# lukedan/libfluid

Hardware: AMD Instinct MI355X
Metric: particle_steps_per_sec (higher is better)
Workload: dtype f32

## Files before the change

libfluid_amd/csrc/common.h:

```cpp
#pragma once

#include <hip/hip_runtime.h>
#include <stdint.h>

#include <string>
#include <vector>

#include "../../include/libfluid_amd.h"

hipError_t lfa_pool_malloc(void **p, size_t bytes);
hipError_t lfa_pool_free(void *p);
void lfa_pool_nosync_begin();
void lfa_pool_nosync_end();
template <typename T> inline hipError_t lfa_hip_malloc(T **p, size_t bytes) { return lfa_pool_malloc((void **)p, bytes); }
#define hipMalloc(p, n) lfa_hip_malloc((p), (n))
#define hipFree(p) lfa_pool_free((void *)(p))
struct lfa_stream_set;
lfa_stream_set *lfa_pool_take_set(int device);
void lfa_pool_park_set(lfa_stream_set *q);

#define LFA_TILE 8
#define LFA_TILE_CELLS 512
#define LFA_HALO 10
#define LFA_HALO_CELLS 1000
// ... 34 lines not shown
	int mg_no_closed = 0;
	int mg_no_tagged = 0;
};

struct lfa_sim {
	int device = 0;
	lfa_knobs knobs;
	hipStream_t stream = nullptr;
	hipStream_t stream2 = nullptr;
	hipEvent_t ev_fork = nullptr, ev_join = nullptr;
	hipStream_t stream3 = nullptr;
	hipEvent_t ev_cfork = nullptr, ev_cjoin = nullptr;
	bool overlap_correction = true;
	bool corr_in_flight = false;
	bool counts_fresh = false;
	bool move_pending = false;
	bool corr_begun = false;
	bool corr_undo_valid = false;
	uint32_t *corr_ovf = nullptr;
	int corr_parts_tiles = 0;
	GridDims g{};
	size_t nc = 0, ncp = 0;
	lfa_params prm{};
	std::string err;

	size_t np = 0, pcap = 0;
	ParticleSoA pb[2];
	int cur = 0;
	uint32_t *rank = nullptr;
	bool binned = false;
// ... 352 lines not shown

int lfa_exclusive_scan_u32(lfa_sim *s, const uint32_t *in, uint32_t *out, size_t n, uint32_t *total_dev);
enum {
	LFA_PIN_SOURCE_TOTAL = 96,
	LFA_PIN_SEED_ACCEPTED = 97,
	LFA_PIN_SEED_OWNED = 98,
	LFA_PIN_RESIDENT = 99,
	LFA_PIN_SOURCE_TOTAL_ALL = 104,
	LFA_PIN_SOURCE_KEPT = 105,
	LFA_PIN_SAMPLE_OWNED = 106,
	LFA_PIN_SAMPLE_OUTSIDE = 107,
};
int lfa_scan_total(lfa_sim *s, const uint32_t *in, uint32_t *out, size_t n, uint32_t *total_dev, int slot, size_t *total);

int lfa_particles_alloc(lfa_sim *s, size_t n);
int lfa_hash_particles_impl(lfa_sim *s, bool counts_done);
int lfa_particles_materialize(lfa_sim *s);
int lfa_c_home_restore(lfa_sim *s);
int lfa_c_home_ensure(lfa_sim *s, size_t n);
int lfa_ensure_io(lfa_sim *s, size_t bytes);
int lfa_slab_download_slots(lfa_sim *s, const uint32_t **slot);
int lfa_sample_velocity_launch(lfa_sim *s, hipStream_t stream, const double *xyz, size_t n, const uint32_t *tile_rule, int z_lo, int z_hi,
                               double *velocity, uint8_t *types, uint32_t *counts_dev);
int lfa_sample_refresh(lfa_sim *s, const char *who, size_t room_bytes, const uint32_t **tile_rule, void **room, int *z_lo, int *z_hi);
int lfa_pcg_alloc(lfa_sim *s);
int lfa_number_unknowns(lfa_sim *s);

__host__ __device__ inline int lfa_stage_index(int hx, int hy, int hz) {
	return (unsigned)(hx - 1) < 8u ? (hx - 1) + 8 * (hy + 10 * hz) : 800 + (hx ? 100 : 0) + hy + 10 * hz;
}
__host__ __device__ inline int lfa_stage_source(int o) {
// ... 64 lines not shown
```

libfluid_amd/csrc/core.hip:

```cpp
#include <math.h>

#include <algorithm>
#include <stdarg.h>
#include <stdio.h>
#include <string.h>

#include <mutex>

#include "common.h"
#include "pcg.h"
#include "stream_set.h"

static thread_local std::string g_create_error;

int lfa_fail(lfa_sim *s, int code, const char *fmt, ...) {
	char buf[512];
	va_list ap;
	va_start(ap, fmt);
	vsnprintf(buf, sizeof buf, fmt, ap);
	va_end(ap);
	if (s) s->err = buf;
	else g_create_error = buf;
	return code;
}
// ... 1033 lines not shown

int lfa_particles_materialize(lfa_sim *s) {
	if (!s->vc_pending) return LFA_OK;
	LFA_TRY(lfa_corr_commit(s));
	s->vc_pending = false;
	LFA_HIP(s, hipSetDevice(s->device));
	const size_t n = s->np_live;
	if (!n) return LFA_OK;
	hipLaunchKernelGGL(k_gather_vc, dim3((unsigned)((n + 255) / 256)), dim3(256), 0, s->stream, n, s->pb[s->cur ^ 1], s->pb[s->cur],
	                   (const uint32_t *)s->vc_src, s->vc_with_c ? 1 : 0);
	LFA_LAUNCH_CHECK(s);
	return LFA_OK;
}

extern "C" int lfa_hash_particles(lfa_sim *s) { return lfa_hash_particles_impl(s, false); }
int lfa_hash_particles_impl(lfa_sim *s, bool counts_done) {
	if (!s) return LFA_E_INVALID;
	LFA_HIP(s, hipSetDevice(s->device));
	LFA_TRY(lfa_corr_commit(s));
	LFA_TRY(lfa_particles_materialize(s));
	const GridDims &g = s->g;
	const int nt = g.nt, L = g.ntx * g.nty;
	const size_t n = s->binned ? s->np_live : s->np;
	ParticleSoA &src = s->pb[s->cur], &dst = s->pb[s->cur ^ 1];
	const int own_lo = s->slab_lo * L, own_hi = s->slab_hi * L;
	const int all_lo = lfa_has_lo(s) ? own_lo - L : own_lo, all_hi = lfa_has_hi(s) ? own_hi + L : own_hi;

	if (!counts_done) {
		LFA_HIP(s, hipMemsetAsync(s->tile_count, 0, (size_t)(nt + 1) * 4, s->stream));
		if (n) {
			hipLaunchKernelGGL(k_tile_count, dim3((unsigned)((n + 256 * TC_CHUNKS - 1) / (256 * TC_CHUNKS))), dim3(256), 0, s->stream, src.key, n,
			                   s->tile_count, s->rank);
			LFA_LAUNCH_CHECK(s);
		}
	}
	LFA_TRY(lfa_exclusive_scan_u32(s, s->tile_count, s->tile_start, (size_t)nt + 1, nullptr));
	LFA_HIP(s, hipMemcpyAsync(s->h_pinned + 8, s->tile_start + nt, 4, hipMemcpyDeviceToHost, s->stream));

	hipLaunchKernelGGL(k_tile_flags, dim3((nt + 255) / 256), dim3(256), 0, s->stream, s->tile_count, s->tile_flag, nt);
	LFA_LAUNCH_CHECK(s);
	LFA_TRY(lfa_dist_exchange_tile_layers_u32(s, s->tile_flag));
	hipLaunchKernelGGL(k_fill_i32, dim3((nt + 255) / 256), dim3(256), 0, s->stream, s->tile_pslot, nt, -1);
	LFA_LAUNCH_CHECK(s);
	const bool one_sync = !s->dist;
	if (one_sync) {
		uint32_t *tot = (uint32_t *)s->pcg_state + 8;
		LFA_TRY(compact_tiles_async(s, s->tile_flag, 0, nt, s->ptiles_all, s->tile_pslot, tot));
		LFA_HIP(s, hipMemsetAsync(s->tile_flag, 0, (size_t)(nt + 1) * 4, s->stream));
		hipLaunchKernelGGL(k_dilate_slots, dim3((nt + 255) / 256), dim3(256), 0, s->stream, (const int *)s->tile_pslot, s->tile_flag, g);
		LFA_LAUNCH_CHECK(s);
		LFA_TRY(compact_tiles_async(s, s->tile_flag, 0, nt, s->dtiles, nullptr, tot + 1));
		LFA_HIP(s, hipMemcpyAsync(s->h_pinned + 9, tot, 8, hipMemcpyDeviceToHost, s->stream));
		LFA_HIP(s, hipStreamSynchronize(s->stream));
		s->n_ptiles_all = (int)s->h_pinned[9];
		s->n_dtiles = (int)s->h_pinned[10];
		s->p_off = 0;
		s->n_ptiles = s->n_ptiles_all;
		s->n_own_first = s->n_own_last = s->n_ghost_lo = s->n_ghost_hi = 0;
		s->ptiles = s->ptiles_all;
	} else {
		uint32_t *tot = (uint32_t *)s->pcg_state + 20;
		LFA_TRY(compact_tiles_async(s, s->tile_flag, all_lo, all_hi, s->ptiles_all, s->tile_pslot, tot));
		int marks[4] = {own_lo, own_lo + L < own_hi ? own_lo + L : own_hi, own_hi - L > own_lo ? own_hi - L : own_lo, own_hi};
		int *didx = s->pcg_state + 12;
		LFA_HIP(s, hipMemcpyAsync(didx, marks, 16, hipMemcpyHostToDevice, s->stream));
		hipLaunchKernelGGL(k_gather_u32, dim3(1), dim3(64), 0, s->stream, s->tile_scan, didx, 4, tot + 1);
		LFA_LAUNCH_CHECK(s);
		LFA_HIP(s, hipMemsetAsync(s->tile_flag, 0, (size_t)(nt + 1) * 4, s->stream));
		hipLaunchKernelGGL(k_dilate_slots, dim3((nt + 255) / 256), dim3(256), 0, s->stream, (const int *)s->tile_pslot, s->tile_flag, g);
		LFA_LAUNCH_CHECK(s);
		if (own_lo > 0) LFA_HIP(s, hipMemsetAsync(s->tile_flag, 0, (size_t)own_lo * 4, s->stream));
		if (own_hi < nt) LFA_HIP(s, hipMemsetAsync(s->tile_flag + own_hi, 0, (size_t)(nt - own_hi) * 4, s->stream));
		LFA_TRY(lfa_dist_exchange_tile_layers_u32(s, s->tile_flag));
		LFA_TRY(compact_tiles_async(s, s->tile_flag, own_lo, own_hi, s->dtiles, nullptr, tot + 5));
		{
// ... 12 lines not shown
		s->p_off = vals[0];
		s->n_ptiles = vals[3] - vals[0];
		s->n_own_first = vals[1] - vals[0];
		s->n_own_last = vals[3] - vals[2];
		s->n_ghost_lo = s->p_off;
		s->n_ghost_hi = s->n_ptiles_all - vals[3];
		s->ptiles = s->ptiles_all + s->p_off;
		s->n_dtiles = (int)h[5];
		for (int w = 0; w < 4; ++w) s->n_halo[w] = (int)h[6 + w];
	}
	s->np_live = s->h_pinned[8];
	if (s->dist) s->np = s->np_live;
	s->holes = false;
	s->n_arrivals = 0;
	s->move_pending = false;
	if (n) {
		const dim3 sgrid((unsigned)((n + 255) / 256));
		const bool home = s->prm.simulation_method != LFA_APIC;
		if (home && !s->c_home_valid) {
			LFA_TRY(lfa_c_home_ensure(s, s->dist ? std::max<size_t>(s->pcap, (size_t)s->next_global_id) : s->pcap));
			hipLaunchKernelGGL(k_c_to_home, sgrid, dim3(256), 0, s->stream, n, src, s->c_home, s->c_home_cap);
			LFA_LAUNCH_CHECK(s);
			s->c_home_valid = true;
		} else if (!home && s->c_home_valid) {
			LFA_TRY(lfa_c_home_restore(s));
		}
		hipLaunchKernelGGL(k_tile_scatter, sgrid, dim3(256), 0, s->stream, n, src, dst, s->rank, s->tile_start, s->tile_count,
		                   s->binned ? 0 : 1, s->vc_src);
		LFA_LAUNCH_CHECK(s);
		s->cur ^= 1;
		s->vc_pending = true;
		s->vc_extent = n;
		s->vc_with_c = !home;
	}
	if (s->n_dtiles) {
		int grid = s->n_dtiles < 8192 ? s->n_dtiles : 8192;
		hipLaunchKernelGGL(k_cell_count, dim3(grid), dim3(256), 0, s->stream, s->dtiles, s->n_dtiles,
		                   s->pb[s->cur].key, s->tile_start, s->cell_count);
		LFA_LAUNCH_CHECK(s);
	}
	s->binned = true;
	s->system_valid = false;
	s->unknown_count_valid = false;
	return LFA_OK;
}

int lfa_dist_build_halo_lists(lfa_sim *s, const uint32_t *flag, int *lists, int n[4]) {
	const int L = s->g.ntx * s->g.nty;
	const int lo[4] = {s->slab_lo * L, (s->slab_hi - 1) * L, (s->slab_lo - 1) * L, s->slab_hi * L};
	const bool on[4] = {lfa_has_lo(s), lfa_has_hi(s), lfa_has_lo(s), lfa_has_hi(s)};
	uint32_t *tot = (uint32_t *)s->pcg_state + 26;
	LFA_HIP(s, hipMemsetAsync(tot, 0, 16, s->stream));
	for (int w = 0; w < 4; ++w)
		if (on[w]) LFA_TRY(compact_tiles_async(s, flag, lo[w], lo[w] + L, lists + (size_t)w * L, nullptr, tot + w));
	LFA_HIP(s, hipMemcpyAsync(s->h_pinned + 26, tot, 16, hipMemcpyDeviceToHost, s->stream));
// ... 3 lines not shown
}

__global__ void k_raw_unknown_flags(GridDims g, size_t nc, const uint32_t *cell_count, const uint32_t *tile_flag,
                                    uint32_t *flag, int z0, int z1) {
	size_t r = (size_t)blockIdx.x * blockDim.x + threadIdx.x;
	if (r >= nc) return;
	int x = (int)(r % g.nx), y = (int)((r / g.nx) % g.ny), z = (int)(r / ((size_t)g.nx * g.ny));
	uint32_t b = blocked_index(g, x, y, z);
	flag[r] = (z >= z0 && z < z1 && tile_flag[b >> 9] && cell_count[b] > 0) ? 1u : 0u;
}

int lfa_number_unknowns(lfa_sim *s) {
	if (s->unknown_count_valid) return LFA_OK;
	if (!s->binned) return lfa_fail(s, LFA_E_INVALID, "call lfa_hash_particles first");
	if (!s->raw_scan) LFA_HIP(s, hipMalloc(&s->raw_scan, (s->nc + 1) * 4));
	hipLaunchKernelGGL(k_raw_unknown_flags, dim3((unsigned)((s->nc + 255) / 256)), dim3(256), 0, s->stream, s->g, s->nc,
	                   s->cell_count, s->tile_flag, s->raw_scan, s->slab_lo * 8, s->slab_hi * 8);
	LFA_LAUNCH_CHECK(s);
	LFA_TRY(lfa_exclusive_scan_u32(s, s->raw_scan, s->raw_scan, s->nc, (uint32_t *)s->pcg_state + 10));
	LFA_HIP(s, hipMemcpyAsync(s->h_pinned, (uint32_t *)s->pcg_state + 10, 4, hipMemcpyDeviceToHost, s->stream));
	LFA_HIP(s, hipStreamSynchronize(s->stream));
	s->n_unknowns = s->h_pinned[0];
	s->unknown_count_valid = true;
	return LFA_OK;
}

extern "C" uint64_t lfa_num_fluid_cells(lfa_sim *s) {
	if (!s || lfa_number_unknowns(s) != LFA_OK) return 0;
	return s->n_unknowns;
}
// ... 24 lines not shown

__global__ void k_export_counts(GridDims g, size_t nc, const uint32_t *cell_count, const uint32_t *tile_flag,
                                uint32_t *out) {
	size_t r = (size_t)blockIdx.x * blockDim.x + threadIdx.x;
	if (r >= nc) return;
	int x = (int)(r % g.nx), y = (int)((r / g.nx) % g.ny), z = (int)(r / ((size_t)g.nx * g.ny));
	uint32_t b = blocked_index(g, x, y, z);
	out[r] = tile_flag[b >> 9] ? cell_count[b] : 0u;
}

extern "C" int lfa_download_cell_counts(lfa_sim *s, uint32_t *count) {
	if (!s || !count) return LFA_E_INVALID;
	if (!s->binned) return lfa_fail(s, LFA_E_INVALID, "call lfa_hash_particles first");
	LFA_HIP(s, hipSetDevice(s->device));
	LFA_TRY(lfa_ensure_io(s, s->nc * 4));
	hipLaunchKernelGGL(k_export_counts, dim3((unsigned)((s->nc + 255) / 256)), dim3(256), 0, s->stream, s->g, s->nc,
	                   s->cell_count, s->tile_flag, (uint32_t *)s->io_buf);
	LFA_LAUNCH_CHECK(s);
	LFA_HIP(s, hipMemcpyAsync(count, s->io_buf, s->nc * 4, hipMemcpyDeviceToHost, s->stream));
	LFA_HIP(s, hipStreamSynchronize(s->stream));
	return LFA_OK;
}

__global__ void __launch_bounds__(256) k_max_speed2(size_t n, const float *vx, const float *vy, const float *vz, double *partials) {
	__shared__ double lds[4];
	double m = 0.0;
	for (size_t i = (size_t)blockIdx.x * 256 + threadIdx.x; i < n; i += (size_t)gridDim.x * 256) {
		double x = vx[i], y = vy[i], z = vz[i];
		double l = x * x + y * y + z * z;
		m = l > m ? l : m;
// ... 174 lines not shown
```

libfluid_amd/csrc/grid_ops.hip:

```cpp
#include "common.h"
#include "pcg.h"

namespace {

struct GridView {
	GridDims g;
	const uint8_t *ctype, *solid;
	const uint32_t *cell_count, *tile_flag;
};
__device__ inline bool is_unknown_at(const GridView &gv, int x, int y, int z) {
	if (!in_grid(gv.g, x, y, z)) return false;
	uint32_t b = blocked_index(gv.g, x, y, z);
	return gv.tile_flag[b >> 9] && gv.cell_count[b] > 0;
}

#define HT_UNKNOWN 8
__device__ inline void stage_halo_types(const GridView &gv, int tx, int ty, int tz, uint8_t *H) {
	for (int i = threadIdx.x; i < LFA_HALO_CELLS; i += 256) {
		const int x = 8 * tx + i % 10 - 1, y = 8 * ty + (i / 10) % 10 - 1, z = 8 * tz + i / 100 - 1;
		uint8_t t = CT_SOLID;
		if (in_grid(gv.g, x, y, z)) {
			const uint32_t b = blocked_index(gv.g, x, y, z);
			if (gv.tile_flag[b >> 9]) t = (uint8_t)((gv.ctype[b] & 7) | (gv.cell_count[b] > 0 ? HT_UNKNOWN : 0));
			else t = gv.solid[b] ? CT_SOLID : CT_AIR;
// ... 399 lines not shown
		f[n] = s->ctype; e[n++] = 1;
		f[n] = s->cell_count; e[n++] = 4;
		if (s->prm.simulation_method == LFA_FLIP_BLEND && s->uo) {
			f[n] = s->uo; e[n++] = 4;
			f[n] = s->vo; e[n++] = 4;
			f[n] = s->wo; e[n++] = 4;
		}
	}
	return lfa_dist_exchange_fields(s, n, f, e);
}
static GridView make_view(lfa_sim *s) { return GridView{s->g, s->ctype, s->solid, s->cell_count, s->tile_flag}; }

int lfa_build_rhs(lfa_sim *s, double dt) {
	if (!s->binned) return lfa_fail(s, LFA_E_INVALID, "lfa_build_system: call lfa_hash_particles first");
	LFA_TRY(lfa_pcg_alloc(s));
	LFA_TRY(lfa_dist_refresh_grid(s, true));
	s->a_scale = dt / (s->prm.density * s->prm.cell_size * s->prm.cell_size);
	s->sys_dt = dt;
	if (!s->n_ptiles) return LFA_OK;
	GridView gv = make_view(s);
	if (!s->tile_closed) {
		LFA_HIP(s, hipMalloc(&s->tile_closed, (size_t)s->g.nt));
		LFA_HIP(s, hipMemsetAsync(s->tile_closed, 0, (size_t)s->g.nt, s->stream));
	}
	hipLaunchKernelGGL(k_abits, dim3(grid_blocks(s->n_ptiles)), dim3(256), 0, s->stream, s->ptiles, s->n_ptiles, gv,
	                   s->abits, s->tile_closed);
	LFA_LAUNCH_CHECK(s);
	const int G = pcg_grid_uncapped(s->n_ptiles);
	const float inv_h = (float)(1.0 / s->prm.cell_size);
	if (!s->tile_epoch) {
// ... 9 lines not shown
		hipLaunchKernelGGL(k_rhs<double>, dim3(G), dim3(256), 0, s->stream, s->ptiles, s->n_ptiles, gv, s->u, s->v, s->w,
		                   (double *)s->vr, (double *)s->vp, inv_h, s->partials + PART_B2, s->tile_epoch, keep_epoch, s->solve_epoch);
	else
		hipLaunchKernelGGL(k_rhs<float>, dim3(G), dim3(256), 0, s->stream, s->ptiles, s->n_ptiles, gv, s->u, s->v, s->w,
		                   (float *)s->vr, (float *)s->vp, inv_h, s->partials + PART_B2, s->tile_epoch, keep_epoch, s->solve_epoch);
	LFA_LAUNCH_CHECK(s);
	return LFA_OK;
}

extern "C" int lfa_apply_pressure(lfa_sim *s, double dt) {
	if (!s) return LFA_E_INVALID;
	if (!s->binned || !s->vp) return lfa_fail(s, LFA_E_INVALID, "lfa_apply_pressure: no pressure on the device");
	LFA_HIP(s, hipSetDevice(s->device));
	if (s->dist) LFA_TRY(lfa_dist_exchange_slices(s, s->vp, s->prm.pcg_dtype == LFA_PCG_F64 ? 8 : 4));
	if (!s->n_dtiles) return LFA_OK;
	const float coeff = (float)(dt / (s->prm.density * s->prm.cell_size));
	GridView gv = make_view(s);
	dim3 grid(grid_blocks(s->n_dtiles));
	if (s->prm.pcg_dtype == LFA_PCG_F64)
		hipLaunchKernelGGL(k_apply_pressure<double>, grid, dim3(256), 0, s->stream, s->dtiles, s->n_dtiles, gv, s->u, s->v,
		                   s->w, (const double *)s->vp, coeff);
	else
		hipLaunchKernelGGL(k_apply_pressure<float>, grid, dim3(256), 0, s->stream, s->dtiles, s->n_dtiles, gv, s->u, s->v,
		                   s->w, (const float *)s->vp, coeff);
	LFA_LAUNCH_CHECK(s);
	return LFA_OK;
}

extern "C" int lfa_extrapolate(lfa_sim *s) {
	if (!s) return LFA_E_INVALID;
	if (!s->binned) return lfa_fail(s, LFA_E_INVALID, "lfa_extrapolate: call lfa_hash_particles first");
	LFA_HIP(s, hipSetDevice(s->device));
	const int iters = (int)s->prm.velocity_extrapolation_iterations;
	if (iters == 0) return LFA_OK;
	LFA_TRY(lfa_dist_refresh_grid(s, false));
	if (!s->n_dtiles) return LFA_OK;
	GridView gv = make_view(s);
	dim3 grid(grid_blocks(s->n_dtiles));
	if (iters == 1) {
		hipLaunchKernelGGL(k_extrapolate, grid, dim3(256), 0, s->stream, s->dtiles, s->n_dtiles, gv, s->u, s->v, s->w,
		                   (const uint8_t *)nullptr, (uint8_t *)nullptr);
		LFA_LAUNCH_CHECK(s);
		return LFA_OK;
	}
	LFA_TRY(lfa_pcg_alloc(s));
	uint8_t *va = (uint8_t *)s->vq, *vb = va + s->ncp;
	for (int i = 0; i < iters; ++i) {
		hipLaunchKernelGGL(k_extrapolate, grid, dim3(256), 0, s->stream, s->dtiles, s->n_dtiles, gv, s->u, s->v, s->w,
		                   i == 0 ? (const uint8_t *)nullptr : (const uint8_t *)va, vb);
		LFA_LAUNCH_CHECK(s);
		uint8_t *t = va; va = vb; vb = t;
// ... 63 lines not shown
```

libfluid_amd/csrc/p2g.hip:

```cpp
#include "common.h"

namespace {

__device__ inline void axis_bf(float t, bool own, int &b, float &f) {
	if (own) {
		b = t >= 1.0f ? 0 : -1;
		f = t >= 1.0f ? 0.0f : t;
	} else {
		b = t < 0.5f ? -1 : 0;
		f = t < 0.5f ? t + 0.5f : t - 0.5f;
	}
}

template <bool APIC, bool QUIRK, typename AddFn>
__device__ inline void scatter_particle(int lx, int ly, int lz, const float t[3], const float v[3], const float c[9],
                                        float hworld, int rot, AddFn add) {
	if (QUIRK) {
#pragma unroll
		for (int comp = 0; comp < 3; ++comp) {
			float w1[3][3], a1[3][3];
			const float *cc = c + 3 * comp;
#pragma unroll
			for (int a = 0; a < 3; ++a)
#pragma unroll
// ... 105 lines not shown
	r.key = p.key[i];
#pragma unroll
	for (int k = 0; k < 3; ++k) {
		r.t[k] = p.t[k][i];
		r.v[k] = pvc.v[k][j];
	}
	if (APIC) {
#pragma unroll
		for (int k = 0; k < 9; ++k) r.c[k] = pvc.c[k][j];
	}
}

#ifndef P2G_THREADS
#define P2G_THREADS 512
#endif
template <bool APIC, bool QUIRK>
__global__ void __launch_bounds__(P2G_THREADS)
k_p2g_binned(const int *ptiles, int n_ptiles, ParticleSoA p, ParticleSoA pvc, const uint32_t *from, const uint32_t *tile_start,
             float *stage, float hworld, int rot_mask) {
	__shared__ unsigned long long acc[6 * LFA_HALO_CELLS];
	for (int slot = blockIdx.x; slot < n_ptiles; slot += gridDim.x) {
		const int tile = ptiles[slot];
		for (int i = threadIdx.x; i < 6 * LFA_HALO_CELLS; i += P2G_THREADS) acc[i] = 0ull;
		__syncthreads();
		const uint32_t beg = tile_start[tile], end = tile_start[tile + 1];
		ParticleRegs cur, nxt;
		uint32_t i = beg + threadIdx.x;
		uint32_t jn = i + P2G_THREADS < end ? (from ? from[i + P2G_THREADS] : i + P2G_THREADS) : 0u;
		if (i < end) load_particle<APIC>(p, pvc, i, from ? from[i] : i, cur);
		for (; i < end; i += P2G_THREADS) {
			const uint32_t in = i + P2G_THREADS;
			const uint32_t jnn = in + P2G_THREADS < end ? (from ? from[in + P2G_THREADS] : in + P2G_THREADS) : 0u;
			if (in < end) load_particle<APIC>(p, pvc, in, jn, nxt);
			jn = jnn;
			const int l = (int)(cur.key & 511);
			if (!QUIRK)
				scatter_particle_lds<APIC>(acc, l & 7, (l >> 3) & 7, l >> 6, cur.t, cur.v, cur.c, hworld, (int)(threadIdx.x & rot_mask));
			else
				scatter_particle<APIC, QUIRK>(l & 7, (l >> 3) & 7, l >> 6, cur.t, cur.v, cur.c, hworld, (int)(threadIdx.x & rot_mask),
				                       [&](int comp, int hx, int hy, int hz, float wv, float wgt) {
					                       unsigned long long *a = acc + comp * 2 * LFA_HALO_CELLS + hx + 10 * hy + 100 * hz;
					                       atomicAdd(a, to_fixed(wv, P2G_FIX_SCALE_V));
					                       atomicAdd(a + LFA_HALO_CELLS, to_fixed(wgt, P2G_FIX_SCALE_W));
				                       });
			cur = nxt;
		}
		__syncthreads();
		float *out = stage + (size_t)slot * 6 * LFA_HALO_CELLS;
		for (int k = threadIdx.x; k < 6 * LFA_HALO_CELLS; k += P2G_THREADS) {
			const int ch = k / LFA_HALO_CELLS;
			out[k] = (float)((double)(long long)acc[ch * LFA_HALO_CELLS + lfa_stage_source(k - ch * LFA_HALO_CELLS)] *
			                 ((ch & 1) ? 1.0 / P2G_FIX_SCALE_W : 1.0 / P2G_FIX_SCALE_V));
		}
		__syncthreads();
	}
}

__global__ void k_zero_acc(const int *dtiles, int n_dtiles, float *acc, size_t ncp) {
	int slot = blockIdx.x;
	if (slot >= n_dtiles) return;
	size_t base = (size_t)dtiles[slot] * LFA_TILE_CELLS;
	for (int k = 0; k < 6; ++k) {
		acc[k * ncp + base + threadIdx.x] = 0.0f;
		acc[k * ncp + base + 256 + threadIdx.x] = 0.0f;
	}
}

template <bool APIC, bool QUIRK>
// ... 14 lines not shown
		for (int k = 0; k < 9; ++k) c[k] = p.c[k][i];
	}
	scatter_particle<APIC, QUIRK>(0, 0, 0, t, v, c, hworld, 0, [&](int comp, int hx, int hy, int hz, float wv, float wgt) {
		int x = cx + hx - 1, y = cy + hy - 1, z = cz + hz - 1;
		if (!in_grid(g, x, y, z)) return;
		size_t b = blocked_index(g, x, y, z);
		unsafeAtomicAdd(acc + (size_t)(2 * comp) * ncp + b, wv);
		unsafeAtomicAdd(acc + (size_t)(2 * comp + 1) * ncp + b, wgt);
	});
}

struct FinalizeParams {
	int method;
	float g[3];
	int fuse_gravity;
};

template <bool BINNED>
__global__ void __launch_bounds__(256)
k_p2g_finalize(const int *dtiles, int n_dtiles, GridDims g, const int *tile_pslot, const float *stage, const float *acc,
               size_t ncp, const uint32_t *cell_count, const uint8_t *solid, float *u, float *v, float *w, float *uo,
               float *vo, float *wo, uint8_t *ctype, FinalizeParams fp) {
	__shared__ int ps27[27];
	for (int slot = blockIdx.x; slot < n_dtiles; slot += gridDim.x) {
		const int tile = dtiles[slot];
		int tx, ty, tz;
		tile_coords(g, tile, tx, ty, tz);
		if (BINNED) {
			__syncthreads();
			if (threadIdx.x < 27) {
				const int nx_ = tx + (int)threadIdx.x % 3 - 1, ny_ = ty + ((int)threadIdx.x / 3) % 3 - 1, nz_ = tz + (int)threadIdx.x / 9 - 1;
				const bool in = (unsigned)nx_ < (unsigned)g.ntx && (unsigned)ny_ < (unsigned)g.nty && (unsigned)nz_ < (unsigned)g.ntz;
				ps27[threadIdx.x] = in ? tile_pslot[nx_ + g.ntx * (ny_ + g.nty * nz_)] : -1;
			}
			__syncthreads();
		}
#pragma unroll
		for (int half = 0; half < 2; ++half) {
			const int l = threadIdx.x + 256 * half;
			const int lx = l & 7, ly = (l >> 3) & 7, lz = l >> 6;
			const size_t b = (size_t)tile * LFA_TILE_CELLS + l;
			const int x = tx * 8 + lx, y = ty * 8 + ly, z = tz * 8 + lz;
			float s[6] = {0.f, 0.f, 0.f, 0.f, 0.f, 0.f};
			if (BINNED) {
				const int ox0 = lx == 0 ? -1 : 0, ox1 = lx == 7 ? 1 : 0, oy0 = ly == 0 ? -1 : 0, oy1 = ly == 7 ? 1 : 0;
				const int oz0 = lz == 0 ? -1 : 0, oz1 = lz == 7 ? 1 : 0;
				for (int oz = oz0; oz <= oz1; ++oz)
					for (int oy = oy0; oy <= oy1; ++oy)
						for (int ox = ox0; ox <= ox1; ++ox) {
							const int ps = ps27[(ox + 1) + 3 * (oy + 1) + 9 * (oz + 1)];
							if (ps < 0) continue;
							const float *src = stage + (size_t)ps * 6 * LFA_HALO_CELLS + lfa_stage_index(lx - 8 * ox + 1, ly - 8 * oy + 1, lz - 8 * oz + 1);
#pragma unroll
							for (int k = 0; k < 6; ++k) s[k] += src[k * LFA_HALO_CELLS];
						}
			} else {
#pragma unroll
				for (int k = 0; k < 6; ++k) s[k] = acc[(size_t)k * ncp + b];
			}
			const bool inside = in_grid(g, x, y, z);
			float vel[3];
#pragma unroll
			for (int k = 0; k < 3; ++k) vel[k] = s[2 * k + 1] > 1e-6f ? s[2 * k] / s[2 * k + 1] : 0.0f;
			uint8_t type;
			if (!inside) {
				vel[0] = vel[1] = vel[2] = 0.0f;
				type = CT_SOLID | CT_OUTSIDE;
			} else if (solid[b]) {
				type = CT_SOLID;
			} else {
				type = cell_count[b] > 0 ? CT_FLUID : CT_AIR;
			}
			const bool bx = x == g.nx - 1, by = y == g.ny - 1, bz = z == g.nz - 1;
			if (fp.method == LFA_FLIP_BLEND && inside) {
				uo[b] = bx ? 0.0f : vel[0];
				vo[b] = by ? 0.0f : vel[1];
				wo[b] = bz ? 0.0f : vel[2];
			}
			if (fp.method == LFA_APIC) {
				if (bx) vel[0] = 0.0f;
				if (by) vel[1] = 0.0f;
				if (bz) vel[2] = 0.0f;
			}
			if (fp.fuse_gravity && inside) {
				vel[0] += fp.g[0]; vel[1] += fp.g[1]; vel[2] += fp.g[2];
			}
// ... 14 lines not shown
			const int l = threadIdx.x + 256 * half;
			if (!in_grid(g, tx * 8 + (l & 7), ty * 8 + ((l >> 3) & 7), tz * 8 + (l >> 6))) continue;
			const size_t b = (size_t)tile * LFA_TILE_CELLS + l;
			u[b] += gx; v[b] += gy; w[b] += gz;
		}
	}
}
}

static int grid_blocks(int n) { return n < 16384 ? (n > 0 ? n : 1) : 16384; }

static int scatter_mode(const lfa_sim *s) {
	if (s->prm.simulation_method != LFA_APIC) return 0;
	return (s->prm.apic_unscaled_kernel && s->prm.cell_size != 1.0) ? 2 : 1;
}
static void launch_binned(lfa_sim *s, const ParticleSoA &p, const ParticleSoA &pvc, const uint32_t *from, float *stage_own) {
	const dim3 grid(grid_blocks(s->n_ptiles));
	const float hworld = (float)s->prm.cell_size;
#define LB(A, Q)                                                                                                             \
	hipLaunchKernelGGL((k_p2g_binned<A, Q>), grid, dim3(P2G_THREADS), 0, s->stream, s->ptiles, s->n_ptiles, p, pvc, from, s->tile_start, \
	                   stage_own, hworld, rot_mask)
	const int rot_mask = 7;
	switch (scatter_mode(s)) {
	case 0: LB(false, false); break;
	case 1: LB(true, false); break;
	default: LB(true, true); break;
	}
#undef LB
}
static void launch_atomic(lfa_sim *s, const ParticleSoA &p) {
	const dim3 grid((unsigned)((s->np_live + 255) / 256));
	const float hworld = (float)s->prm.cell_size;
#define LA(A, Q) hipLaunchKernelGGL((k_p2g_atomic<A, Q>), grid, dim3(256), 0, s->stream, s->np_live, p, s->acc, s->ncp, s->g, hworld)
	switch (scatter_mode(s)) {
	case 0: LA(false, false); break;
	case 1: LA(true, false); break;
	default: LA(true, true); break;
	}
#undef LA
}

int lfa_p2g_run(lfa_sim *s, bool fuse_gravity, double dt) {
	if (!s->binned) return lfa_fail(s, LFA_E_INVALID, "lfa_p2g: call lfa_hash_particles first");
	LFA_HIP(s, hipSetDevice(s->device));
	LFA_TRY(lfa_corr_commit(s));
	const int method = s->prm.simulation_method;
	if (method == LFA_FLIP_BLEND && !s->uo) {
		LFA_HIP(s, hipMalloc(&s->uo, s->ncp * 4));
		LFA_HIP(s, hipMalloc(&s->vo, s->ncp * 4));
		LFA_HIP(s, hipMalloc(&s->wo, s->ncp * 4));
		LFA_HIP(s, hipMemsetAsync(s->uo, 0, s->ncp * 4, s->stream));
		LFA_HIP(s, hipMemsetAsync(s->vo, 0, s->ncp * 4, s->stream));
		LFA_HIP(s, hipMemsetAsync(s->wo, 0, s->ncp * 4, s->stream));
	}
	const bool binned = s->prm.p2g_variant == LFA_P2G_LDS_BINNED;
	if (!binned) LFA_TRY(lfa_particles_materialize(s));
	const ParticleSoA &p = s->pb[s->cur], &pvc = s->vc_pending ? s->pb[s->cur ^ 1] : s->pb[s->cur];
	const uint32_t *from = s->vc_pending ? (const uint32_t *)s->vc_src : (const uint32_t *)nullptr;
	if (s->timing) LFA_HIP(s, hipEventRecord(s->ev[16], s->stream));
	if (binned) {
		if ((size_t)s->n_ptiles_all > s->stage_tiles) {
			if (s->stage) LFA_HIP(s, hipFree(s->stage));
			s->stage = nullptr;
			size_t want = (size_t)s->n_ptiles_all + (size_t)s->n_ptiles_all / 4 + 16;
			hipError_t e = hipMalloc(&s->stage, want * 6 * LFA_HALO_CELLS * 4);
			if (e != hipSuccess) return lfa_fail(s, LFA_E_OOM, "hipMalloc of the P2G staging slabs (%zu tiles) failed", want);
			s->stage_tiles = want;
		}
		if (s->n_ptiles) {
			launch_binned(s, p, pvc, from, s->stage + (size_t)s->p_off * 6 * LFA_HALO_CELLS);
			LFA_LAUNCH_CHECK(s);
			if (from) ++s->stat_p2g_deferred;
		}
		LFA_TRY(lfa_dist_exchange_p2g_planes(s, s->stage));
	} else {
		if (s->dist) return lfa_fail(s, LFA_E_UNSUPPORTED, "the global-atomic P2G variant is single-GPU only");
		if (!s->acc) {
			hipError_t e = hipMalloc(&s->acc, s->ncp * 6 * 4);
			if (e != hipSuccess) return lfa_fail(s, LFA_E_OOM, "hipMalloc of the atomic P2G accumulators failed");
		}
		if (s->n_dtiles) {
			hipLaunchKernelGGL(k_zero_acc, dim3(s->n_dtiles), dim3(256), 0, s->stream, s->dtiles, s->n_dtiles, s->acc,
			                   s->ncp);
			LFA_LAUNCH_CHECK(s);
		}
		if (s->np_live) {
			launch_atomic(s, p);
			LFA_LAUNCH_CHECK(s);
		}
	}
	if (s->timing) LFA_HIP(s, hipEventRecord(s->ev[17], s->stream));
	FinalizeParams fp;
	fp.method = method;
	fp.fuse_gravity = fuse_gravity ? 1 : 0;
	for (int k = 0; k < 3; ++k) fp.g[k] = fuse_gravity ? (float)(s->prm.gravity[k] * dt) : 0.0f;
	if (s->n_dtiles) {
		dim3 grid(grid_blocks(s->n_dtiles));
		if (binned)
			hipLaunchKernelGGL(k_p2g_finalize<true>, grid, dim3(256), 0, s->stream, s->dtiles, s->n_dtiles, s->g,
			                   s->tile_pslot, s->stage, s->acc, s->ncp, s->cell_count, s->solid, s->u, s->v, s->w, s->uo,
			                   s->vo, s->wo, s->ctype, fp);
		else
			hipLaunchKernelGGL(k_p2g_finalize<false>, grid, dim3(256), 0, s->stream, s->dtiles, s->n_dtiles, s->g,
			                   s->tile_pslot, s->stage, s->acc, s->ncp, s->cell_count, s->solid, s->u, s->v, s->w, s->uo,
			                   s->vo, s->wo, s->ctype, fp);
		LFA_LAUNCH_CHECK(s);
	}
	LFA_HIP(s, hipMemcpyAsync(s->grid_flag, s->tile_flag, (size_t)s->g.nt * 4, hipMemcpyDeviceToDevice, s->stream));
	s->grid_valid = true;
// ... 28 lines not shown
	if (which == LFA_K_P2G_SCATTER) {
		if (s->prm.p2g_variant == LFA_P2G_LDS_BINNED) {
			if (!s->stage || (size_t)s->n_ptiles_all > s->stage_tiles) return lfa_fail(s, LFA_E_INVALID, "no staging slabs");
			launch_binned(s, p, pvc, from, s->stage + (size_t)s->p_off * 6 * LFA_HALO_CELLS);
		} else {
			if (!s->acc) return lfa_fail(s, LFA_E_INVALID, "no accumulators");
			launch_atomic(s, p);
		}
		LFA_LAUNCH_CHECK(s);
		return LFA_OK;
	}
	if (which == LFA_K_P2G_FINALIZE) {
		FinalizeParams fp;
		fp.method = s->prm.simulation_method;
		fp.fuse_gravity = 0;
		fp.g[0] = fp.g[1] = fp.g[2] = 0.f;
		dim3 grid(grid_blocks(s->n_dtiles));
		if (s->prm.p2g_variant == LFA_P2G_LDS_BINNED)
			hipLaunchKernelGGL(k_p2g_finalize<true>, grid, dim3(256), 0, s->stream, s->dtiles, s->n_dtiles, s->g,
			                   s->tile_pslot, s->stage, s->acc, s->ncp, s->cell_count, s->solid, s->u, s->v, s->w, s->uo,
			                   s->vo, s->wo, s->ctype, fp);
		else
			hipLaunchKernelGGL(k_p2g_finalize<false>, grid, dim3(256), 0, s->stream, s->dtiles, s->n_dtiles, s->g,
			                   s->tile_pslot, s->stage, s->acc, s->ncp, s->cell_count, s->solid, s->u, s->v, s->w, s->uo,
			                   s->vo, s->wo, s->ctype, fp);
		LFA_LAUNCH_CHECK(s);
		return LFA_OK;
	}
	if (which == LFA_K_BIN) return lfa_hash_particles(s);
	return lfa_fail(s, LFA_E_INVALID, "unknown kernel id %d", which);
// ... 2 lines not shown
```

libfluid_amd/csrc/particles.hip:

```cpp
#include <math.h>

#include <algorithm>
#include <utility>

#include "common.h"
#include "pcg.h"

namespace {

__device__ inline bool solid_or_outside(const GridDims &g, const uint8_t *solid, int x, int y, int z) {
	if (!in_grid(g, x, y, z)) return true;
	return solid[blocked_index(g, x, y, z)] != 0;
}

__device__ inline void collide(const GridDims &g, const uint8_t *solid, double from[3], double to[3], double skin) {
	for (int bounce = 0; bounce < 3; ++bounce) {
		bool hit = false;
		double diff[3], inv[3], t[3];
		int cur[3], last[3], adv[3];
#pragma unroll
		for (int d = 0; d < 3; ++d) {
			cur[d] = (int)floor(from[d]);
			last[d] = (int)floor(to[d]);
			diff[d] = to[d] - from[d];
// ... 1013 lines not shown
			LFA_HIP(s, hipMemcpy(q.cell, k_cell.data(), nk * 4, hipMemcpyHostToDevice));
			LFA_HIP(s, hipMemcpy(q.of, k_of.data(), nk * 4, hipMemcpyHostToDevice));
			LFA_HIP(s, hipMemcpy(q.gidx, k_g.data(), nk * 4, hipMemcpyHostToDevice));
			LFA_HIP(s, hipMemcpy(q.mode, k_mode.data(), nk * 4, hipMemcpyHostToDevice));
		}
		q.n_cand = nk;
		q.n_global = ng;
	}
	s->sources_built = s->sources;
	s->sources_valid = true;
	return LFA_OK;
}

static int source_needs(lfa_sim *s) {
	const size_t n = s->n_src_entries;
	hipLaunchKernelGGL(k_source_need, dim3((unsigned)((n + 255) / 256)), dim3(256), 0, s->stream, (const uint32_t *)s->src_cell,
	                   (const uint32_t *)s->src_lo, (const uint32_t *)s->src_target, n, (const uint32_t *)s->cell_count,
	                   (const uint32_t *)s->tile_flag, s->src_need);
	LFA_LAUNCH_CHECK(s);
	return LFA_OK;
}

static int source_room(lfa_sim *s, size_t base, size_t count, uint64_t id_lo, size_t id_n, size_t id_end, const double *positions,
                       uint64_t positions_capacity, const char *keeps) {
	if (base + count >= ((size_t)1 << 32)) return lfa_fail(s, LFA_E_INVALID, "more than 2^32 particles");
	if (positions && positions_capacity < count)
		return lfa_fail(s, LFA_E_INVALID, "lfa_update_sources_rng: room for %llu positions but %s%zu particles",
		                (unsigned long long)positions_capacity, keeps, count);
	if (positions) LFA_TRY(lfa_ensure_io(s, count * 24));
	LFA_TRY(lfa_particles_materialize(s));
// ... 453 lines not shown
	LFA_HIP(s, hipSetDevice(s->device));
	LFA_TRY(lfa_corr_commit(s));
	const bool tm = s->timing;
	enum { B_START = 24, B_ADVECT, B_BIN, B_P2G, B_SOLVE, B_APPLY, B_CORRECT, B_EXTRAP, B_G2P, B_JOIN };
	static_assert(B_CORRECT == LFA_EV_CORRECT_END, "event slot of the end of the correction");
	auto rec = [&](int id) -> int {
		if (tm) LFA_HIP(s, hipEventRecord(s->ev[id], s->stream));
		return LFA_OK;
	};
	LFA_TRY(rec(B_START));
	LFA_TRY(advect_collide(s, dt, true));
	LFA_TRY(rec(B_ADVECT));
	{
		const bool counted = s->counts_fresh;
		s->counts_fresh = false;
		LFA_TRY(lfa_hash_particles_impl(s, counted));
	}
	if (!s->sources.empty()) LFA_TRY(lfa_update_sources(s, nullptr));
	LFA_TRY(rec(B_BIN));
	const bool overlap = s->overlap_correction && (s->dist || s->np_live);
	LFA_TRY(lfa_p2g_run(s, true, dt));
	LFA_TRY(rec(B_P2G));
	if (overlap) {
		if (s->dist) LFA_TRY(lfa_dist_exchange_ghost_particles(s));
		LFA_TRY(correct_begin(s, dt, true));
	}
	double res = 0.0;
	uint64_t it = 0;
	int rc = LFA_OK;
	auto grid_stages = [&]() -> int {
		rc = lfa_pcg_solve(s, dt, &res, &it);
// ... 102 lines not shown
```

libfluid_amd/csrc/pcg.hip:

```cpp
#include "pcg.h"

#include <math.h>
#include <string.h>

#include <stdlib.h>

#include <algorithm>

namespace {

#define WAVE_SYNC() asm volatile("s_waitcnt lgkmcnt(0)" ::: "memory")

template <typename real> struct Vecs {
	real *p, *r, *z, *s, *pre, *q;
};

struct TileCtx {
	const int *ptiles;
	int n_ptiles;
	const int *tile_pslot;
	GridDims g;
};

__device__ inline void face_neighbours(const TileCtx &tc, int tile, int nb[6]) {
// ... 1953 lines not shown
	NEED_SYSTEM(s);
	if (!v || !out) return LFA_E_INVALID;
	return F64(s) ? apply_a_t<double>(s, v, out, n) : apply_a_t<float>(s, v, out, n);
}

static int ev_rec(lfa_sim *s, int i) {
	if (s->timing) LFA_HIP(s, hipEventRecord(s->ev[i], s->stream));
	return LFA_OK;
}

extern "C" int lfa_step_hot(lfa_sim *s, double dt, double *residual, uint64_t *iterations) {
	if (!s) return LFA_E_INVALID;
	LFA_HIP(s, hipSetDevice(s->device));
	LFA_TRY(lfa_corr_commit(s));
	LFA_TRY(ev_rec(s, 0));
	LFA_TRY(lfa_hash_particles(s));
	LFA_TRY(ev_rec(s, 1));
	LFA_TRY(lfa_p2g_run(s, true, dt));
	LFA_TRY(ev_rec(s, 2));
	LFA_TRY(ev_rec(s, 3));
	LFA_TRY(lfa_pcg_alloc(s));
	LFA_TRY(ev_rec(s, 4));
	double res = 0.0;
	uint64_t it = 0;
	int rc = lfa_pcg_solve(s, dt, &res, &it);
	if (rc < 0) return rc;
	LFA_TRY(ev_rec(s, 5));
	LFA_TRY(lfa_apply_pressure(s, dt));
	LFA_TRY(ev_rec(s, 6));
	LFA_TRY(lfa_extrapolate(s));
	LFA_TRY(ev_rec(s, 7));
// ... 145 lines not shown
```

Before: 5.122 billion.

## Overlap tile-list compaction with scatter and fuse cell counting into P2G

In single-device mode, the tile flag, compaction and dilation work now runs on a second stream while the main stream launches the particle scatter, so the host sync no longer serialises both. Per-cell particle counting is deferred during a time step and folded into the binned P2G kernel via LDS atomics, and the finalize kernel zeroes counts for empty dilated tiles. The separate cell-count pass is removed from the hot path. This adds lazy-ensure calls at every consumer of cell counts, extra LDS use, and a waves-per-EU attribute that could change occupancy.

```diff
diff --git a/libfluid_amd/csrc/common.h b/libfluid_amd/csrc/common.h
--- a/libfluid_amd/csrc/common.h
+++ b/libfluid_amd/csrc/common.h
@@ -72,6 +72,7 @@
 	bool overlap_correction = true;
 	bool corr_in_flight = false;
 	bool counts_fresh = false;
+	bool cell_count_pending = false;
 	bool move_pending = false;
 	bool corr_begun = false;
 	bool corr_undo_valid = false;
@@ -454,7 +455,8 @@
 int lfa_scan_total(lfa_sim *s, const uint32_t *in, uint32_t *out, size_t n, uint32_t *total_dev, int slot, size_t *total);
 
 int lfa_particles_alloc(lfa_sim *s, size_t n);
-int lfa_hash_particles_impl(lfa_sim *s, bool counts_done);
+int lfa_hash_particles_impl(lfa_sim *s, bool counts_done, bool in_step = false);
+int lfa_cell_counts_ensure(lfa_sim *s);
 int lfa_particles_materialize(lfa_sim *s);
 int lfa_c_home_restore(lfa_sim *s);
 int lfa_c_home_ensure(lfa_sim *s, size_t n);
diff --git a/libfluid_amd/csrc/core.hip b/libfluid_amd/csrc/core.hip
--- a/libfluid_amd/csrc/core.hip
+++ b/libfluid_amd/csrc/core.hip
@@ -1071,15 +1071,58 @@
 }
 
 extern "C" int lfa_hash_particles(lfa_sim *s) { return lfa_hash_particles_impl(s, false); }
-int lfa_hash_particles_impl(lfa_sim *s, bool counts_done) {
+
+static int launch_cell_count(lfa_sim *s) {
+	if (!s->n_dtiles) return LFA_OK;
+	int grid = s->n_dtiles < 8192 ? s->n_dtiles : 8192;
+	hipLaunchKernelGGL(k_cell_count, dim3(grid), dim3(256), 0, s->stream, s->dtiles, s->n_dtiles,
+	                   s->pb[s->cur].key, s->tile_start, s->cell_count);
+	LFA_LAUNCH_CHECK(s);
+	return LFA_OK;
+}
+int lfa_cell_counts_ensure(lfa_sim *s) {
+	if (!s->cell_count_pending) return LFA_OK;
+	s->cell_count_pending = false;
+	if (!s->binned) return LFA_OK;
+	LFA_HIP(s, hipSetDevice(s->device));
+	return launch_cell_count(s);
+}
+
+static int scatter_prepare(lfa_sim *s, size_t n) {
+	if (!n) return LFA_OK;
+	const bool home = s->prm.simulation_method != LFA_APIC;
+	if (home && !s->c_home_valid) {
+		LFA_TRY(lfa_c_home_ensure(s, s->dist ? std::max<size_t>(s->pcap, (size_t)s->next_global_id) : s->pcap));
+		hipLaunchKernelGGL(k_c_to_home, dim3((unsigned)((n + 255) / 256)), dim3(256), 0, s->stream, n, s->pb[s->cur], s->c_home, s->c_home_cap);
+		LFA_LAUNCH_CHECK(s);
+		s->c_home_valid = true;
+	} else if (!home && s->c_home_valid) {
+		LFA_TRY(lfa_c_home_restore(s));
+	}
+	return LFA_OK;
+}
+static int scatter_launch(lfa_sim *s, size_t n) {
+	if (!n) return LFA_OK;
+	hipLaunchKernelGGL(k_tile_scatter, dim3((unsigned)((n + 255) / 256)), dim3(256), 0, s->stream, n, s->pb[s->cur], s->pb[s->cur ^ 1], s->rank,
+	                   s->tile_start, s->tile_count, s->binned ? 0 : 1, s->vc_src);
+	LFA_LAUNCH_CHECK(s);
+	s->cur ^= 1;
+	s->vc_pending = true;
+	s->vc_extent = n;
+	s->vc_with_c = s->prm.simulation_method == LFA_APIC;
+	return LFA_OK;
+}
+
+int lfa_hash_particles_impl(lfa_sim *s, bool counts_done, bool in_step) {
 	if (!s) return LFA_E_INVALID;
 	LFA_HIP(s, hipSetDevice(s->device));
 	LFA_TRY(lfa_corr_commit(s));
 	LFA_TRY(lfa_particles_materialize(s));
+	s->cell_count_pending = false;
 	const GridDims &g = s->g;
 	const int nt = g.nt, L = g.ntx * g.nty;
 	const size_t n = s->binned ? s->np_live : s->np;
-	ParticleSoA &src = s->pb[s->cur], &dst = s->pb[s->cur ^ 1];
+	ParticleSoA &src = s->pb[s->cur];
 	const int own_lo = s->slab_lo * L, own_hi = s->slab_hi * L;
 	const int all_lo = lfa_has_lo(s) ? own_lo - L : own_lo, all_hi = lfa_has_hi(s) ? own_hi + L : own_hi;
 
@@ -1094,21 +1137,37 @@
 	LFA_TRY(lfa_exclusive_scan_u32(s, s->tile_count, s->tile_start, (size_t)nt + 1, nullptr));
 	LFA_HIP(s, hipMemcpyAsync(s->h_pinned + 8, s->tile_start + nt, 4, hipMemcpyDeviceToHost, s->stream));
 
-	hipLaunchKernelGGL(k_tile_flags, dim3((nt + 255) / 256), dim3(256), 0, s->stream, s->tile_count, s->tile_flag, nt);
-	LFA_LAUNCH_CHECK(s);
-	LFA_TRY(lfa_dist_exchange_tile_layers_u32(s, s->tile_flag));
-	hipLaunchKernelGGL(k_fill_i32, dim3((nt + 255) / 256), dim3(256), 0, s->stream, s->tile_pslot, nt, -1);
-	LFA_LAUNCH_CHECK(s);
 	const bool one_sync = !s->dist;
 	if (one_sync) {
-		uint32_t *tot = (uint32_t *)s->pcg_state + 8;
-		LFA_TRY(compact_tiles_async(s, s->tile_flag, 0, nt, s->ptiles_all, s->tile_pslot, tot));
-		LFA_HIP(s, hipMemsetAsync(s->tile_flag, 0, (size_t)(nt + 1) * 4, s->stream));
-		hipLaunchKernelGGL(k_dilate_slots, dim3((nt + 255) / 256), dim3(256), 0, s->stream, (const int *)s->tile_pslot, s->tile_flag, g);
-		LFA_LAUNCH_CHECK(s);
-		LFA_TRY(compact_tiles_async(s, s->tile_flag, 0, nt, s->dtiles, nullptr, tot + 1));
-		LFA_HIP(s, hipMemcpyAsync(s->h_pinned + 9, tot, 8, hipMemcpyDeviceToHost, s->stream));
-		LFA_HIP(s, hipStreamSynchronize(s->stream));
+		LFA_TRY(scatter_prepare(s, n));
+		LFA_HIP(s, hipEventRecord(s->ev_fork, s->stream));
+		LFA_HIP(s, hipStreamWaitEvent(s->stream2, s->ev_fork, 0));
+		hipStream_t main_stream = s->stream;
+		s->stream = s->stream2;
+		auto lists = [&]() -> int {
+			uint32_t *tot = (uint32_t *)s->pcg_state + 8;
+			hipLaunchKernelGGL(k_tile_flags, dim3((nt + 255) / 256), dim3(256), 0, s->stream, s->tile_count, s->tile_flag, nt);
+			LFA_LAUNCH_CHECK(s);
+			hipLaunchKernelGGL(k_fill_i32, dim3((nt + 255) / 256), dim3(256), 0, s->stream, s->tile_pslot, nt, -1);
+			LFA_LAUNCH_CHECK(s);
+			LFA_TRY(compact_tiles_async(s, s->tile_flag, 0, nt, s->ptiles_all, s->tile_pslot, tot));
+			LFA_HIP(s, hipMemsetAsync(s->tile_flag, 0, (size_t)(nt + 1) * 4, s->stream));
+			hipLaunchKernelGGL(k_dilate_slots, dim3((nt + 255) / 256), dim3(256), 0, s->stream, (const int *)s->tile_pslot, s->tile_flag, g);
+			LFA_LAUNCH_CHECK(s);
+			LFA_TRY(compact_tiles_async(s, s->tile_flag, 0, nt, s->dtiles, nullptr, tot + 1));
+			LFA_HIP(s, hipMemcpyAsync(s->h_pinned + 9, tot, 8, hipMemcpyDeviceToHost, s->stream));
+			return LFA_OK;
+		};
+		int rc = lists();
+		s->stream = main_stream;
+		const hipError_t e_join = hipEventRecord(s->ev_join, s->stream2);
+		if (rc == LFA_OK && e_join == hipSuccess) rc = scatter_launch(s, n);
+		const hipError_t e_host = e_join == hipSuccess ? hipEventSynchronize(s->ev_join) : hipStreamSynchronize(s->stream2);
+		const hipError_t e_wait = e_join == hipSuccess ? hipStreamWaitEvent(s->stream, s->ev_join, 0) : hipSuccess;
+		if (rc < 0) return rc;
+		LFA_HIP(s, e_join);
+		LFA_HIP(s, e_host);
+		LFA_HIP(s, e_wait);
 		s->n_ptiles_all = (int)s->h_pinned[9];
 		s->n_dtiles = (int)s->h_pinned[10];
 		s->p_off = 0;
@@ -1116,6 +1175,11 @@
 		s->n_own_first = s->n_own_last = s->n_ghost_lo = s->n_ghost_hi = 0;
 		s->ptiles = s->ptiles_all;
 	} else {
+		hipLaunchKernelGGL(k_tile_flags, dim3((nt + 255) / 256), dim3(256), 0, s->stream, s->tile_count, s->tile_flag, nt);
+		LFA_LAUNCH_CHECK(s);
+		LFA_TRY(lfa_dist_exchange_tile_layers_u32(s, s->tile_flag));
+		hipLaunchKernelGGL(k_fill_i32, dim3((nt + 255) / 256), dim3(256), 0, s->stream, s->tile_pslot, nt, -1);
+		LFA_LAUNCH_CHECK(s);
 		uint32_t *tot = (uint32_t *)s->pcg_state + 20;
 		LFA_TRY(compact_tiles_async(s, s->tile_flag, all_lo, all_hi, s->ptiles_all, s->tile_pslot, tot));
 		int marks[4] = {own_lo, own_lo + L < own_hi ? own_lo + L : own_hi, own_hi - L > own_lo ? own_hi - L : own_lo, own_hi};
@@ -1158,31 +1222,14 @@
 	s->holes = false;
 	s->n_arrivals = 0;
 	s->move_pending = false;
-	if (n) {
-		const dim3 sgrid((unsigned)((n + 255) / 256));
-		const bool home = s->prm.simulation_method != LFA_APIC;
-		if (home && !s->c_home_valid) {
-			LFA_TRY(lfa_c_home_ensure(s, s->dist ? std::max<size_t>(s->pcap, (size_t)s->next_global_id) : s->pcap));
-			hipLaunchKernelGGL(k_c_to_home, sgrid, dim3(256), 0, s->stream, n, src, s->c_home, s->c_home_cap);
-			LFA_LAUNCH_CHECK(s);
-			s->c_home_valid = true;
-		} else if (!home && s->c_home_valid) {
-			LFA_TRY(lfa_c_home_restore(s));
-		}
-		hipLaunchKernelGGL(k_tile_scatter, sgrid, dim3(256), 0, s->stream, n, src, dst, s->rank, s->tile_start, s->tile_count,
-		                   s->binned ? 0 : 1, s->vc_src);
-		LFA_LAUNCH_CHECK(s);
-		s->cur ^= 1;
-		s->vc_pending = true;
-		s->vc_extent = n;
-		s->vc_with_c = !home;
-	}
-	if (s->n_dtiles) {
-		int grid = s->n_dtiles < 8192 ? s->n_dtiles : 8192;
-		hipLaunchKernelGGL(k_cell_count, dim3(grid), dim3(256), 0, s->stream, s->dtiles, s->n_dtiles,
-		                   s->pb[s->cur].key, s->tile_start, s->cell_count);
-		LFA_LAUNCH_CHECK(s);
-	}
+	if (!one_sync) {
+		LFA_TRY(scatter_prepare(s, n));
+		LFA_TRY(scatter_launch(s, n));
+	}
+	if (in_step && one_sync && s->prm.p2g_variant == LFA_P2G_LDS_BINNED && s->sources.empty())
+		s->cell_count_pending = s->n_dtiles > 0;
+	else
+		LFA_TRY(launch_cell_count(s));
 	s->binned = true;
 	s->system_valid = false;
 	s->unknown_count_valid = false;
@@ -1216,6 +1263,7 @@
 	if (s->unknown_count_valid) return LFA_OK;
 	if (!s->binned) return lfa_fail(s, LFA_E_INVALID, "call lfa_hash_particles first");
 	if (!s->raw_scan) LFA_HIP(s, hipMalloc(&s->raw_scan, (s->nc + 1) * 4));
+	LFA_TRY(lfa_cell_counts_ensure(s));
 	hipLaunchKernelGGL(k_raw_unknown_flags, dim3((unsigned)((s->nc + 255) / 256)), dim3(256), 0, s->stream, s->g, s->nc,
 	                   s->cell_count, s->tile_flag, s->raw_scan, s->slab_lo * 8, s->slab_hi * 8);
 	LFA_LAUNCH_CHECK(s);
@@ -1270,6 +1318,7 @@
 	if (!s->binned) return lfa_fail(s, LFA_E_INVALID, "call lfa_hash_particles first");
 	LFA_HIP(s, hipSetDevice(s->device));
 	LFA_TRY(lfa_ensure_io(s, s->nc * 4));
+	LFA_TRY(lfa_cell_counts_ensure(s));
 	hipLaunchKernelGGL(k_export_counts, dim3((unsigned)((s->nc + 255) / 256)), dim3(256), 0, s->stream, s->g, s->nc,
 	                   s->cell_count, s->tile_flag, (uint32_t *)s->io_buf);
 	LFA_LAUNCH_CHECK(s);
diff --git a/libfluid_amd/csrc/grid_ops.hip b/libfluid_amd/csrc/grid_ops.hip
--- a/libfluid_amd/csrc/grid_ops.hip
+++ b/libfluid_amd/csrc/grid_ops.hip
@@ -437,6 +437,7 @@
 int lfa_build_rhs(lfa_sim *s, double dt) {
 	if (!s->binned) return lfa_fail(s, LFA_E_INVALID, "lfa_build_system: call lfa_hash_particles first");
 	LFA_TRY(lfa_pcg_alloc(s));
+	LFA_TRY(lfa_cell_counts_ensure(s));
 	LFA_TRY(lfa_dist_refresh_grid(s, true));
 	s->a_scale = dt / (s->prm.density * s->prm.cell_size * s->prm.cell_size);
 	s->sys_dt = dt;
@@ -476,6 +477,7 @@
 	LFA_HIP(s, hipSetDevice(s->device));
 	if (s->dist) LFA_TRY(lfa_dist_exchange_slices(s, s->vp, s->prm.pcg_dtype == LFA_PCG_F64 ? 8 : 4));
 	if (!s->n_dtiles) return LFA_OK;
+	LFA_TRY(lfa_cell_counts_ensure(s));
 	const float coeff = (float)(dt / (s->prm.density * s->prm.cell_size));
 	GridView gv = make_view(s);
 	dim3 grid(grid_blocks(s->n_dtiles));
@@ -497,6 +499,7 @@
 	if (iters == 0) return LFA_OK;
 	LFA_TRY(lfa_dist_refresh_grid(s, false));
 	if (!s->n_dtiles) return LFA_OK;
+	LFA_TRY(lfa_cell_counts_ensure(s));
 	GridView gv = make_view(s);
 	dim3 grid(grid_blocks(s->n_dtiles));
 	if (iters == 1) {
diff --git a/libfluid_amd/csrc/p2g.hip b/libfluid_amd/csrc/p2g.hip
--- a/libfluid_amd/csrc/p2g.hip
+++ b/libfluid_amd/csrc/p2g.hip
@@ -143,14 +143,17 @@
 #ifndef P2G_THREADS
 #define P2G_THREADS 512
 #endif
-template <bool APIC, bool QUIRK>
-__global__ void __launch_bounds__(P2G_THREADS)
+template <bool APIC, bool QUIRK, bool COUNT>
+__global__ void __launch_bounds__(P2G_THREADS) __attribute__((amdgpu_waves_per_eu(QUIRK ? 5 : 6)))
 k_p2g_binned(const int *ptiles, int n_ptiles, ParticleSoA p, ParticleSoA pvc, const uint32_t *from, const uint32_t *tile_start,
-             float *stage, float hworld, int rot_mask) {
-	__shared__ unsigned long long acc[6 * LFA_HALO_CELLS];
+             float *stage, float hworld, int rot_mask, uint32_t *cell_count) {
+	__shared__ unsigned long long acc[6 * LFA_HALO_CELLS + (COUNT ? LFA_TILE_CELLS / 2 : 0)];
+	uint32_t *cnt = (uint32_t *)(acc + 6 * LFA_HALO_CELLS);
 	for (int slot = blockIdx.x; slot < n_ptiles; slot += gridDim.x) {
 		const int tile = ptiles[slot];
 		for (int i = threadIdx.x; i < 6 * LFA_HALO_CELLS; i += P2G_THREADS) acc[i] = 0ull;
+		if (COUNT)
+			for (int i = threadIdx.x; i < LFA_TILE_CELLS; i += P2G_THREADS) cnt[i] = 0u;
 		__syncthreads();
 		const uint32_t beg = tile_start[tile], end = tile_start[tile + 1];
 		ParticleRegs cur, nxt;
@@ -172,6 +175,7 @@
 					                       atomicAdd(a, to_fixed(wv, P2G_FIX_SCALE_V));
 					                       atomicAdd(a + LFA_HALO_CELLS, to_fixed(wgt, P2G_FIX_SCALE_W));
 				                       });
+			if (COUNT) atomicAdd(&cnt[cur.key & 511], 1u);
 			cur = nxt;
 		}
 		__syncthreads();
@@ -181,6 +185,8 @@
 			out[k] = (float)((double)(long long)acc[ch * LFA_HALO_CELLS + lfa_stage_source(k - ch * LFA_HALO_CELLS)] *
 			                 ((ch & 1) ? 1.0 / P2G_FIX_SCALE_W : 1.0 / P2G_FIX_SCALE_V));
 		}
+		if (COUNT)
+			for (int i = threadIdx.x; i < LFA_TILE_CELLS; i += P2G_THREADS) cell_count[(size_t)tile * LFA_TILE_CELLS + i] = cnt[i];
 		__syncthreads();
 	}
 }
@@ -225,12 +231,13 @@
 	int method;
 	float g[3];
 	int fuse_gravity;
+	int counts_from_scatter;
 };
 
 template <bool BINNED>
 __global__ void __launch_bounds__(256)
 k_p2g_finalize(const int *dtiles, int n_dtiles, GridDims g, const int *tile_pslot, const float *stage, const float *acc,
-               size_t ncp, const uint32_t *cell_count, const uint8_t *solid, float *u, float *v, float *w, float *uo,
+               size_t ncp, uint32_t *cell_count, const uint8_t *solid, float *u, float *v, float *w, float *uo,
                float *vo, float *wo, uint8_t *ctype, FinalizeParams fp) {
 	__shared__ int ps27[27];
 	for (int slot = blockIdx.x; slot < n_dtiles; slot += gridDim.x) {
@@ -246,11 +253,13 @@
 			}
 			__syncthreads();
 		}
+		const bool empty_tile = BINNED && fp.counts_from_scatter && ps27[13] < 0;
 #pragma unroll
 		for (int half = 0; half < 2; ++half) {
 			const int l = threadIdx.x + 256 * half;
 			const int lx = l & 7, ly = (l >> 3) & 7, lz = l >> 6;
 			const size_t b = (size_t)tile * LFA_TILE_CELLS + l;
+			if (empty_tile) cell_count[b] = 0u;
 			const int x = tx * 8 + lx, y = ty * 8 + ly, z = tz * 8 + lz;
 			float s[6] = {0.f, 0.f, 0.f, 0.f, 0.f, 0.f};
 			if (BINNED) {
@@ -280,7 +289,7 @@
 			} else if (solid[b]) {
 				type = CT_SOLID;
 			} else {
-				type = cell_count[b] > 0 ? CT_FLUID : CT_AIR;
+				type = !empty_tile && cell_count[b] > 0 ? CT_FLUID : CT_AIR;
 			}
 			const bool bx = x == g.nx - 1, by = y == g.ny - 1, bz = z == g.nz - 1;
 			if (fp.method == LFA_FLIP_BLEND && inside) {
@@ -325,17 +334,21 @@
 	if (s->prm.simulation_method != LFA_APIC) return 0;
 	return (s->prm.apic_unscaled_kernel && s->prm.cell_size != 1.0) ? 2 : 1;
 }
-static void launch_binned(lfa_sim *s, const ParticleSoA &p, const ParticleSoA &pvc, const uint32_t *from, float *stage_own) {
+static void launch_binned(lfa_sim *s, const ParticleSoA &p, const ParticleSoA &pvc, const uint32_t *from, float *stage_own,
+                          bool count = false) {
 	const dim3 grid(grid_blocks(s->n_ptiles));
 	const float hworld = (float)s->prm.cell_size;
-#define LB(A, Q)                                                                                                             \
-	hipLaunchKernelGGL((k_p2g_binned<A, Q>), grid, dim3(P2G_THREADS), 0, s->stream, s->ptiles, s->n_ptiles, p, pvc, from, s->tile_start, \
-	                   stage_own, hworld, rot_mask)
+#define LB(A, Q, C)                                                                                                                     \
+	hipLaunchKernelGGL((k_p2g_binned<A, Q, C>), grid, dim3(P2G_THREADS), 0, s->stream, s->ptiles, s->n_ptiles, p, pvc, from, s->tile_start, \
+	                   stage_own, hworld, rot_mask, s->cell_count)
 	const int rot_mask = 7;
-	switch (scatter_mode(s)) {
-	case 0: LB(false, false); break;
-	case 1: LB(true, false); break;
-	default: LB(true, true); break;
+	switch (scatter_mode(s) * 2 + (count ? 1 : 0)) {
+	case 0: LB(false, false, false); break;
+	case 1: LB(false, false, true); break;
+	case 2: LB(true, false, false); break;
+	case 3: LB(true, false, true); break;
+	case 4: LB(true, true, false); break;
+	default: LB(true, true, true); break;
 	}
 #undef LB
 }
@@ -366,6 +379,9 @@
 	}
 	const bool binned = s->prm.p2g_variant == LFA_P2G_LDS_BINNED;
 	if (!binned) LFA_TRY(lfa_particles_materialize(s));
+	const bool count = binned && !s->dist && s->cell_count_pending;
+	if (count) s->cell_count_pending = false;
+	LFA_TRY(lfa_cell_counts_ensure(s));
 	const ParticleSoA &p = s->pb[s->cur], &pvc = s->vc_pending ? s->pb[s->cur ^ 1] : s->pb[s->cur];
 	const uint32_t *from = s->vc_pending ? (const uint32_t *)s->vc_src : (const uint32_t *)nullptr;
 	if (s->timing) LFA_HIP(s, hipEventRecord(s->ev[16], s->stream));
@@ -379,7 +395,7 @@
 			s->stage_tiles = want;
 		}
 		if (s->n_ptiles) {
-			launch_binned(s, p, pvc, from, s->stage + (size_t)s->p_off * 6 * LFA_HALO_CELLS);
+			launch_binned(s, p, pvc, from, s->stage + (size_t)s->p_off * 6 * LFA_HALO_CELLS, count);
 			LFA_LAUNCH_CHECK(s);
 			if (from) ++s->stat_p2g_deferred;
 		}
@@ -404,6 +420,7 @@
 	FinalizeParams fp;
 	fp.method = method;
 	fp.fuse_gravity = fuse_gravity ? 1 : 0;
+	fp.counts_from_scatter = count ? 1 : 0;
 	for (int k = 0; k < 3; ++k) fp.g[k] = fuse_gravity ? (float)(s->prm.gravity[k] * dt) : 0.0f;
 	if (s->n_dtiles) {
 		dim3 grid(grid_blocks(s->n_dtiles));
@@ -462,6 +479,7 @@
 		FinalizeParams fp;
 		fp.method = s->prm.simulation_method;
 		fp.fuse_gravity = 0;
+		fp.counts_from_scatter = 0;
 		fp.g[0] = fp.g[1] = fp.g[2] = 0.f;
 		dim3 grid(grid_blocks(s->n_dtiles));
 		if (s->prm.p2g_variant == LFA_P2G_LDS_BINNED)
diff --git a/libfluid_amd/csrc/particles.hip b/libfluid_amd/csrc/particles.hip
--- a/libfluid_amd/csrc/particles.hip
+++ b/libfluid_amd/csrc/particles.hip
@@ -1051,6 +1051,7 @@
 
 static int source_needs(lfa_sim *s) {
 	const size_t n = s->n_src_entries;
+	LFA_TRY(lfa_cell_counts_ensure(s));
 	hipLaunchKernelGGL(k_source_need, dim3((unsigned)((n + 255) / 256)), dim3(256), 0, s->stream, (const uint32_t *)s->src_cell,
 	                   (const uint32_t *)s->src_lo, (const uint32_t *)s->src_target, n, (const uint32_t *)s->cell_count,
 	                   (const uint32_t *)s->tile_flag, s->src_need);
@@ -1534,7 +1535,7 @@
 	{
 		const bool counted = s->counts_fresh;
 		s->counts_fresh = false;
-		LFA_TRY(lfa_hash_particles_impl(s, counted));
+		LFA_TRY(lfa_hash_particles_impl(s, counted, true));
 	}
 	if (!s->sources.empty()) LFA_TRY(lfa_update_sources(s, nullptr));
 	LFA_TRY(rec(B_BIN));
diff --git a/libfluid_amd/csrc/pcg.hip b/libfluid_amd/csrc/pcg.hip
--- a/libfluid_amd/csrc/pcg.hip
+++ b/libfluid_amd/csrc/pcg.hip
@@ -1991,7 +1991,7 @@
 	LFA_HIP(s, hipSetDevice(s->device));
 	LFA_TRY(lfa_corr_commit(s));
 	LFA_TRY(ev_rec(s, 0));
-	LFA_TRY(lfa_hash_particles(s));
+	LFA_TRY(lfa_hash_particles_impl(s, false, true));
 	LFA_TRY(ev_rec(s, 1));
 	LFA_TRY(lfa_p2g_run(s, true, dt));
 	LFA_TRY(ev_rec(s, 2));
```

Result: no change. 5.160 billion, median of 6 (+0.7%).
